# om-ai-lab/OmChat

Hardware: AMD Instinct MI355X
Metric: images/sec prefill + decode tokens/sec, OmChat-13B TP=1/8; p50 TTFT (higher is better)
Workload: dtype bf16

## Files before the change

omchat_amd/csrc/attention.hip:

```cpp
#include "kernels.h"

#include "attn_common.h"

namespace {

__device__ __forceinline__ float max3(float a, float b, float c) {
  float r;
  asm("v_max3_f32 %0, %1, %2, %3" : "=v"(r) : "v"(a), "v"(b), "v"(c));
  return r;
}
__device__ __forceinline__ float max2(float a, float b) {
  float r;
  asm("v_max_f32 %0, %1, %2" : "=v"(r) : "v"(a), "v"(b));
  return r;
}
__device__ __forceinline__ float max_xor32_raw(float v) {
  const auto r = __builtin_amdgcn_permlane32_swap(__float_as_uint(v), __float_as_uint(v), false, false);
  return max2(__uint_as_float(r[0]), __uint_as_float(r[1]));
}
__device__ __forceinline__ float max_xor16_raw(float v) {
  const auto r = __builtin_amdgcn_permlane16_swap(__float_as_uint(v), __float_as_uint(v), false, false);
  return max2(__uint_as_float(r[0]), __uint_as_float(r[1]));
}

// ... 507 lines not shown
#pragma unroll
        for (int r = 0; r < 16; ++r) mg[d * 16 + r] = o[d][r];
      mg[DB * 16] = m_run; mg[DB * 16 + 1] = l_run;
    }
    __syncthreads();
    if (kg == 1) return;
    const float m1 = mg[DB * 16], l1 = mg[DB * 16 + 1];
    const float m = max2(m_run, m1);
    const float a0 = __builtin_amdgcn_exp2f((m_run - m) * p.c), a1 = __builtin_amdgcn_exp2f((m1 - m) * p.c);
    l_run = l_run * a0 + l1 * a1;
#pragma unroll
    for (int d = 0; d < DB; ++d)
#pragma unroll
      for (int r = 0; r < 16; ++r) o[d][r] = o[d][r] * a0 + mg[d * 16 + r] * a1;
  }
  const float l = sum_xor32(l_run);
  if (wave_active && qrow < p.Sq) {
    const float inv = l > 0.f ? 1.f / l : 0.f;
    T* op = (T*)p.O + b * p.o_sb + hq * p.o_sh + (int64_t)qrow * p.o_sr + 4 * hh;
#pragma unroll
    for (int db = 0; db < DB; ++db)
#pragma unroll
      for (int g = 0; g < 4; ++g) {
        typename V8<T>::half_type h4;
#pragma unroll
        for (int r = 0; r < 4; ++r) h4[r] = fromf<T>(o[db][4 * g + r] * inv);
        *reinterpret_cast<typename V8<T>::half_type*>(op + db * 32 + g * 8) = h4;
      }
  }
}

template <typename T, bool KV8 = false, bool MASKED = false>
__global__ __launch_bounds__(64, 2) void attn_decode_kernel(AttnP p) {
  __shared__ __attribute__((aligned(256))) char Vs[KV_TILE * 256];
  const int lane = threadIdx.x, fc = lane & 15, fg = lane >> 4;
  const int split = blockIdx.x, kvh = blockIdx.y, b = blockIdx.z;
  const int n_rep = p.q_heads / p.kv_heads, hq0 = kvh * n_rep;
  const int kv_len = p.kv_len ? p.kv_len[b] : p.Skv;
#if OMCHAT_EXPERIMENTS
  if (p.dbg && split < 8 && kvh == 0 && lane == 0) atomicMax(p.dbg + 10, ~wall_clock64());
#endif
  float* wsb = p.ws + ((size_t)(b * p.q_heads + hq0 + (fc < n_rep ? fc : 0)) * p.nsplit + split) * WS_STRIDE;
  if (split * KV_TILE >= kv_len) {
    if (fc < n_rep && fg == 0) { wsb[128] = NEG_BIG; wsb[129] = 0.f; }
    return;
  }
  f32x4 o[8];
  float mx, l;
  attn_decode_tile<T, KV8, false, MASKED>(p, split, kvh, b, kv_len, Vs, lane, o, mx, l);
  if (fc < n_rep) {
#pragma unroll
    for (int dn = 0; dn < 8; ++dn) *reinterpret_cast<f32x4*>(wsb + dn * 16 + fg * 4) = o[dn];
    if (fg == 0) { wsb[128] = mx; wsb[129] = l; }
  }
#if OMCHAT_EXPERIMENTS
  if (p.dbg && kvh == 0 && lane == 0) atomicMax(p.dbg + 11, wall_clock64());
#endif
}

template <typename T, bool KLDS = false>
__global__ __launch_bounds__(64, 2) void attn_decode_multi_kernel(AttnP p) {
  typedef typename V8<T>::type frag_t;
  __shared__ __attribute__((aligned(256))) char Vs[KV_TILE * 256];
  const int lane = threadIdx.x, fc = lane & 15, fg = lane >> 4;
  const int split = blockIdx.x, kvh = blockIdx.y, b = blockIdx.z;
  const int n_rep = p.q_heads / p.kv_heads, hq0 = kvh * n_rep;
  const int kv_len = p.kv_len ? p.kv_len[b] : p.Skv;
  const int key_base = split * KV_TILE * p.tpw;
  float* wsb = p.ws + ((size_t)(b * p.q_heads + hq0 + (fc < n_rep ? fc : 0)) * p.nsplit + split) * WS_STRIDE;
  if (key_base >= kv_len) {
    if (fc < n_rep && fg == 0) { wsb[128] = NEG_BIG; wsb[129] = 0.f; }
    return;
  }
  const bool fuse = p.rope != nullptr;
  const int pp = kv_len - 1;
  const int pt = pp < p.rope_max ? pp : p.rope_max - 1;
  const T* Kg = (const T*)p.K + b * p.k_sb + kvh * p.k_sh;
  const T* Vg = (const T*)p.V + b * p.v_sb + kvh * p.v_sh;
  const T* kn = fuse ? (const T*)p.k_new + b * p.new_sb + kvh * 128 : nullptr;
  const T* vn = fuse ? (const T*)p.v_new + b * p.new_sb + kvh * 128 : nullptr;

  frag_t qf[4];
  {
    const int hh = fc < n_rep ? fc : n_rep - 1;
    const T* qp = (const T*)p.Q + b * p.q_sb + (hq0 + hh) * p.q_sh;
#pragma unroll
    for (int ds = 0; ds < 4; ++ds) qf[ds] = ld8<T>(qp + ds * 32 + fg * 8);
    if (fuse) {
#pragma unroll
      for (int ds = 0; ds < 2; ++ds) {
        const float* cs = p.rope + ((size_t)pt * 64 + ds * 32 + fg * 8) * 2;
        const frag_t lo = qf[ds], hi = qf[ds + 2];
        qf[ds] = rope_chunk<T>(lo, hi, cs, false);
        qf[ds + 2] = rope_chunk<T>(hi, lo, cs, true);
      }
    }
  }
  f32x4 o[8];
#pragma unroll
  for (int dn = 0; dn < 8; ++dn) o[dn] = (f32x4){0.f, 0.f, 0.f, 0.f};
  float m_run = NEG_BIG, l_run = 0.f;
  const int tq = fc >> 2, tp = fc & 3;
  const int vrow_lo = 4 * fg + tq;
  const int vswz = ((vrow_lo & 7) << 1);

  for (int tt = 0; tt < p.tpw; ++tt) {
// ... 790 lines not shown
  __syncthreads();
  if (g == 0) {
    float ltot = red[NWV], tot = part[0][dl];
#pragma unroll
    for (int i = 1; i < NWV; ++i) ltot += red[NWV + i];
#pragma unroll
    for (int i = 1; i < NGRP; ++i) tot += part[i][dl];
    O[pack_nb ? packed_x_index(b, h * 128 + d, pack_nb) : (size_t)(b * o_sb + h * o_sh + d)] = fromf<T>(tot / ltot);
  }
}

template <typename T>
__global__ __launch_bounds__(256) void kv_quant_kernel(const T* kc, const T* vc, unsigned char* k8, unsigned char* v8, float* ks, float* vs, int kv_heads,
                                                       int64_t c_sb, int64_t c_sh, int64_t s_sb, int64_t s_sh, const int* pos_lo, int pos0, const int* len,
                                                       int max_rows) {
  const int lane = threadIdx.x & 63, wave = threadIdx.x >> 6;
  const int r = blockIdx.x * 4 + wave;
  const int h = blockIdx.y, b = blockIdx.z;
  const int lo = pos_lo ? pos_lo[b] : pos0;
  const int pos = lo + r;
  if (r >= max_rows || (len && pos >= len[b])) return;
  const int64_t off = b * c_sb + h * c_sh + (int64_t)pos * 128 + lane * 2;
  const int64_t soff = b * s_sb + h * s_sh + pos;
#pragma unroll
  for (int which = 0; which < 2; ++which) {
    const T* src = (which ? vc : kc) + off;
    const float x0 = tof(src[0]), x1 = tof(src[1]);
    float m = fmaxf(fabsf(x0), fabsf(x1));
    m = wave_max(m);
    const float sc = m > 0.f ? m / 448.0f : 1.0f;
    const int pk = __builtin_amdgcn_cvt_pk_fp8_f32(x0 / sc, x1 / sc, 0, false);
    *reinterpret_cast<unsigned short*>((which ? v8 : k8) + off) = (unsigned short)(pk & 0xFFFF);
    if (lane == 0) (which ? vs : ks)[soff] = sc;
  }
}

}

int launch_kv_quant(int dtype, const void* kc, const void* vc, void* k8, void* v8, float* ks, float* vs, int b, int kv_heads, int64_t c_sb, int64_t c_sh,
                    int64_t s_sb, int64_t s_sh, const int* pos_lo, int pos0, const int* len, int max_rows, hipStream_t s) {
  if (b <= 0 || max_rows <= 0) return 0;
  dim3 grid(cdiv(max_rows, 4), kv_heads, b);
  if (dtype == OMCHAT_F16) hipLaunchKernelGGL(kv_quant_kernel<f16>, grid, dim3(256), 0, s, (const f16*)kc, (const f16*)vc, (unsigned char*)k8, (unsigned char*)v8,
                                              ks, vs, kv_heads, c_sb, c_sh, s_sb, s_sh, pos_lo, pos0, len, max_rows);
  else if (dtype == OMCHAT_BF16) hipLaunchKernelGGL(kv_quant_kernel<bf16>, grid, dim3(256), 0, s, (const bf16*)kc, (const bf16*)vc, (unsigned char*)k8,
                                                    (unsigned char*)v8, ks, vs, kv_heads, c_sb, c_sh, s_sb, s_sh, pos_lo, pos0, len, max_rows);
  else { omchat_set_error("launch_kv_quant: bad dtype"); return 1; }
  OM_LAUNCH_CHECK();
  return 0;
}

int g_attn_kv8_tpw = 0;
void attn_set_kv8_tpw(int v) { g_attn_kv8_tpw = v < 0 || v > 15 ? 0 : v; }
int g_attn_tpw = 0;
void attn_set_tpw(int v) { g_attn_tpw = v < 0 ? 0 : v; }
int g_merge_dg = 1;
void attn_set_merge_dg(int v) { g_merge_dg = v; }
int g_merge_mid_min = 64;
void attn_set_merge_mid_min(int v) { g_merge_mid_min = v < 1 ? 1 : v; }
int g_attn_dma = 1;
void attn_set_dma(int v) { g_attn_dma = v; }
int g_attn_dma_slots = 0;
int g_attn_dma_stages = 2;
void attn_set_dma_slots(int v) { g_attn_dma_slots = v & 255; const int st = (v >> 8) & 255; g_attn_dma_stages = st < 2 ? 2 : (st > 4 ? 4 : st); }
int g_attn_kg = 0;
void attn_set_kg(int v) { g_attn_kg = v; }
template <typename K>
static int launch_attn2(K kern, dim3 grid, int threads, int lds, hipStream_t s, const AttnP& p, PerDeviceOnce* attr_done) {
  if (attr_done->first()) OM_HIP(hipFuncSetAttribute((const void*)kern, hipFuncAttributeMaxDynamicSharedMemorySize, lds));
  hipLaunchKernelGGL(kern, grid, dim3(threads), lds, s, p);
  return 0;
}
#define OM_LAUNCH_ATTN2(KERN, GRID, THREADS, LDS)                                     \
  do { static PerDeviceOnce done_; const int rc_ = launch_attn2((KERN), (GRID), (THREADS), (LDS), s, p, &done_); if (rc_) return rc_; } while (0)
int g_attn_peel = 1;
void attn_set_peel(int v) { g_attn_peel = v; }
int g_attn_mha_xcd = 1;
void attn_set_mha_xcd(int v) { g_attn_mha_xcd = v; }
int g_attn_hsplit = -1;
void attn_set_hsplit(int v) { g_attn_hsplit = v; }
int g_attn_dma_rot = 0;
void attn_set_dma_rot(int v) { g_attn_dma_rot = v; }
int g_attn_klds = 0;
void attn_set_klds(int v) { g_attn_klds = v; }
int g_attn_v2 = 1;
void attn_set_v2(int v) { g_attn_v2 = v; }

namespace {
template <typename T>
__global__ __launch_bounds__(128) void attn_uniform_rows_kernel(AttnP p) {
  const int h = blockIdx.x, b = blockIdx.y, d = threadIdx.x;
  const int start = p.kv_start[b];
  if (start <= 0) return;
  const int kvh = h / (p.q_heads / p.kv_heads);
  const T* V = (const T*)p.V + b * p.v_sb + kvh * p.v_sh + d;
  const float w = rnd<T>(1.0f / (float)p.Skv);
  float acc = 0.f;
  for (int j = 0; j < p.Skv; ++j) acc += w * tof(V[(int64_t)j * p.v_sr]);
  const T o = fromf<T>(acc);
  T* O = (T*)p.O + b * p.o_sb + h * p.o_sh + d;
  for (int i = 0; i < start && i < p.Sq; ++i) O[(int64_t)i * p.o_sr] = o;
}
}

int launch_attn_uniform_rows(int dtype, const AttnArgs& a, hipStream_t s) {
  OM_CHECK(a.kv_start && (a.head_dim == 0 || a.head_dim == 128), "uniform rows: left-padded batch (kv_start), head dim 128");
// ... 101 lines not shown
  return (size_t)batch * q_heads * cdiv(max_len, KV_TILE) * WS_STRIDE * sizeof(float);
}

static void kv8_plan(int batch, int kv_heads, int L, bool masked, int* tpw, int* nw) {
  *tpw = 1; *nw = 1;
  if (masked) return;
  const long waves1 = (long)cdiv(L, KV_TILE) * kv_heads * batch;
  if (g_attn_kv8_tpw > 0) { *tpw = g_attn_kv8_tpw & 7; *nw = (g_attn_kv8_tpw & 8) ? 4 : 1; }
  else {
    *tpw = waves1 >= 2L * device_cus() ? 3 : 1;
    const int n4 = cdiv(L, 12 * KV_TILE);
    if (*tpw == 3 && n4 <= 64 && (long)n4 * kv_heads * batch >= device_cus() / 2) *nw = 4;
  }
  if (*tpw < 1 || *tpw > 4) *tpw = 1;
  if (*tpw != 3) *nw = 1;
}
int g_attn_kv8_fuse = 1;
void attn_set_kv8_fuse(int v) { g_attn_kv8_fuse = v; }
bool attn_decode_kv8_fuses_rope(int batch, int kv_heads, int L, bool masked) {
  int tpw, nw;
  kv8_plan(batch, kv_heads, L, masked, &tpw, &nw);
  const long waves = (long)cdiv(L, KV_TILE * tpw * nw) * nw * kv_heads * batch;
  return g_attn_kv8_fuse && tpw == 3 && waves <= 4L * device_cus();
}

struct MergeDone { unsigned* flags = nullptr; unsigned epoch = 0; int mode = 0; unsigned long long* dbg = nullptr; };
template <typename T>
static void launch_merge(const float* ws, int nsplit, int q_heads, int rows, const int* kv_len, int L, float c, void* O, int64_t o_sb, int64_t o_sh,
                         int pack_nb, int split_keys, hipStream_t s, const MergeDone& done = MergeDone{}) {
  const dim3 mgrid(q_heads, rows);
  if (nsplit > g_merge_mid_min && nsplit <= 256) {
    if (g_merge_dg == 2) hipLaunchKernelGGL((attn_merge_mid_kernel<T, 4, 2>), dim3(q_heads, rows, 2), dim3(512), 0, s, ws, nsplit, q_heads, kv_len, L, c, (T*)O, o_sb, o_sh, pack_nb, split_keys);
    else hipLaunchKernelGGL((attn_merge_mid_kernel<T, 4, 1>), mgrid, dim3(512), 0, s, ws, nsplit, q_heads, kv_len, L, c, (T*)O, o_sb, o_sh, pack_nb, split_keys);
  } else if (nsplit > 256 && nsplit <= 1024) {
    if (g_merge_dg >= 1) hipLaunchKernelGGL((attn_merge_mid_kernel<T, 8, 4>), dim3(q_heads, rows, 4), dim3(1024), 0, s, ws, nsplit, q_heads, kv_len, L, c, (T*)O, o_sb, o_sh, pack_nb, split_keys);
    else hipLaunchKernelGGL((attn_merge_mid_kernel<T, 8, 1>), mgrid, dim3(1024), 0, s, ws, nsplit, q_heads, kv_len, L, c, (T*)O, o_sb, o_sh, pack_nb, split_keys);
  } else {
    hipLaunchKernelGGL(attn_merge_kernel<T>, mgrid, dim3(128), 0, s, ws, nsplit, q_heads, kv_len, L, c, (T*)O, o_sb, o_sh, pack_nb, split_keys,
                       done.flags, done.epoch, done.mode, done.dbg);
  }
}

int launch_attn_merge(int dtype, const float* ws, int nsplit, int q_heads, int rows, const int* kv_len, int L, float scale, void* O, int split_keys,
                      hipStream_t s) {
  OM_CHECK(ws && O && nsplit > 0 && q_heads > 0 && rows > 0 && L > 0 && split_keys > 0, "launch_attn_merge: null or empty argument");
  const float c = scale * 1.4426950408889634f;
  if (dtype == OMCHAT_F16) launch_merge<f16>(ws, nsplit, q_heads, rows, kv_len, L, c, O, (int64_t)q_heads * 128, 128, 0, split_keys, s);
  else if (dtype == OMCHAT_BF16) launch_merge<bf16>(ws, nsplit, q_heads, rows, kv_len, L, c, O, (int64_t)q_heads * 128, 128, 0, split_keys, s);
  else { omchat_set_error("launch_attn_merge: bad dtype"); return 1; }
  OM_LAUNCH_CHECK();
  return 0;
}

struct DecodeForm { bool masked, kv8, kv8_fuse, dma; int tpw, kv8_nw, dma_lds, nsplit, split_keys; };
template <typename T>
static void launch_decode_form(const AttnDecodeArgs& a, const DecodeForm& f, dim3 grid, const AttnP& p, hipStream_t s) {
  if (f.masked && f.kv8) hipLaunchKernelGGL((attn_decode_kernel<T, true, true>), grid, dim3(64), 0, s, p);
  else if (f.masked) hipLaunchKernelGGL((attn_decode_kernel<T, false, true>), grid, dim3(64), 0, s, p);
  else if (f.kv8 && f.tpw == 2) hipLaunchKernelGGL((attn_decode_kv8_walk_kernel<T, 2, 1>), grid, dim3(64), 0, s, p);
  else if (f.kv8_fuse && f.kv8_nw == 4) hipLaunchKernelGGL((attn_decode_kv8_walk_kernel<T, 3, 4, true>), grid, dim3(256), 0, s, p);
  else if (f.kv8_fuse) hipLaunchKernelGGL((attn_decode_kv8_walk_kernel<T, 3, 1, true>), grid, dim3(64), 0, s, p);
  else if (f.kv8 && f.tpw == 3 && f.kv8_nw == 4) hipLaunchKernelGGL((attn_decode_kv8_walk_kernel<T, 3, 4>), grid, dim3(256), 0, s, p);
  else if (f.kv8 && f.tpw == 3) hipLaunchKernelGGL((attn_decode_kv8_walk_kernel<T, 3, 1>), grid, dim3(64), 0, s, p);
  else if (f.kv8 && f.tpw == 4) hipLaunchKernelGGL((attn_decode_kv8_walk_kernel<T, 4, 1>), grid, dim3(64), 0, s, p);
  else if (f.kv8) hipLaunchKernelGGL((attn_decode_kernel<T, true>), grid, dim3(64), 0, s, p);
  else if (f.dma && g_attn_dma_stages == 2) hipLaunchKernelGGL((attn_decode_dma_kernel<T, 2>), grid, dim3(64), f.dma_lds, s, p);
  else if (f.dma && g_attn_dma_stages == 3) hipLaunchKernelGGL((attn_decode_dma_kernel<T, 3>), grid, dim3(64), f.dma_lds, s, p);
  else if (f.dma) hipLaunchKernelGGL((attn_decode_dma_kernel<T, 4>), grid, dim3(64), f.dma_lds, s, p);
  else if (f.tpw > 1 && g_attn_klds) hipLaunchKernelGGL((attn_decode_multi_kernel<T, true>), grid, dim3(64), 0, s, p);
  else if (f.tpw > 1) hipLaunchKernelGGL((attn_decode_multi_kernel<T, false>), grid, dim3(64), 0, s, p);
  else hipLaunchKernelGGL((attn_decode_kernel<T, false>), grid, dim3(64), 0, s, p);
  launch_merge<T>(a.ws, f.nsplit, a.q_heads, a.batch, a.kv_len, a.L, p.c, a.O, a.o_sb, a.o_sh, a.o_pack_nb, f.split_keys, s,
                  MergeDone{a.done_flags, a.done_epoch, a.done_mode, a.done_dbg});
}

int launch_attn_decode(int dtype, const AttnDecodeArgs& a, hipStream_t s) {
  OM_CHECK(a.q_heads % a.kv_heads == 0 && a.q_heads / a.kv_heads <= 16, "group size must be <= 16");
  OM_CHECK(a.L > 0 && a.batch > 0, "empty attention");
  const bool kv8 = a.k_scale != nullptr;
  const long waves1 = (long)cdiv(a.L, KV_TILE) * a.kv_heads * a.batch;
  int tpw = kv8 ? 1 : (waves1 >= 6144 ? 4 : (waves1 >= 3072 ? 2 : 1));
  if (g_attn_tpw > 0 && !kv8) tpw = g_attn_tpw;
  int kv8_nw = 1;
  if (kv8) kv8_plan(a.batch, a.kv_heads, a.L, a.key_mask != nullptr, &tpw, &kv8_nw);
  if (a.key_mask) tpw = 1;
  const long tiles32 = (long)cdiv(a.L, DMA_TILE) * a.kv_heads * a.batch;
  const bool dma = g_attn_dma && !kv8 && !a.key_mask && a.k_sr == 128 && a.v_sr == 128 && (g_attn_tpw > 1 || (g_attn_tpw == 0 && tiles32 >= 6L * device_cus()));
  int dma_slots = g_attn_dma_slots;
  if (!dma_slots) {
    const int pairs = a.kv_heads * a.batch, tpw4 = cdiv(cdiv(a.L, DMA_TILE), std::max(1, 4 * device_cus() / pairs));
    dma_slots = (pairs >= 16 && tpw4 >= 4 && tpw4 <= 8 && tiles32 < 32L * device_cus()) ? 4 : 2;
  }
  int split_keys = KV_TILE * tpw * kv8_nw;
  if (dma) {
    const int slots = dma_slots * device_cus(), pairs = a.kv_heads * a.batch;
    const int tiles = cdiv(a.L, DMA_TILE);
    const int ns_target = std::max(1, slots / pairs);
    tpw = std::max(2, cdiv(tiles, ns_target));
    split_keys = DMA_TILE * tpw;
  }
  const int nsplit = cdiv(a.L, split_keys);
  OM_CHECK(a.ws && a.ws_bytes >= attn_decode_ws_bytes(a.batch, a.q_heads, a.L), "workspace too small");
  AttnP p{a.Q, a.K, a.V, nullptr, a.q_sb, a.q_sh, 0, a.k_sb, a.k_sh, a.k_sr, a.v_sb, a.v_sh, a.v_sr, 0, 0, 0,
          a.kv_len, nullptr, a.q_heads, a.kv_heads, 1, a.L, 0, 0, nsplit, a.scale * 1.4426950408889634f, a.ws,
          a.rope, a.pos, a.k_new, a.v_new, a.new_sb, (void*)a.K, (void*)a.V, a.rope_max, a.k_scale, a.v_scale, a.scale_sb, a.scale_sh, tpw,
          a.key_mask, a.mask_sb};
#if OMCHAT_EXPERIMENTS
  p.dbg = a.done_dbg;
#endif
  OM_CHECK(!a.key_mask || (((kv8 && !a.rope) || (!kv8 && a.rope && a.pos)) && !a.kv_len && a.mask_sb % 64 == 0 && a.mask_sb >= a.L),
           "masked decode: fused RoPE with explicit positions (16-bit cache) or rows appended beforehand (e4m3 cache), uniform length, mask rows padded to a multiple of 64");
  const bool kv8_fuse = kv8 && a.rope != nullptr;
  OM_CHECK(!kv8 || a.v_scale, "fp8 KV cache: both scale arrays");
  OM_CHECK(!kv8_fuse || (tpw == 3 && a.k_new && a.v_new && a.k16_w && a.v16_w && !a.key_mask),
           "fp8 KV cache with fused RoPE: the walking form only (attn_decode_kv8_fuses_rope), raw k / v rows and the 16-bit caches to append to");
  OM_CHECK(!a.rope || (a.k_new && a.v_new), "fused RoPE decode needs k_new and v_new (kv_len == null: every sequence holds exactly L keys)");
  OM_CHECK(a.o_pack_nb == 0 || (a.batch <= 16 * a.o_pack_nb && a.o_sh == 128 && a.q_heads % 1 == 0), "packed output: batch <= 16 * NB, head stride 128");
  if (kv8_fuse) { p.k_cache_w = a.k16_w; p.v_cache_w = a.v16_w; }
  if (dma) p.causal = g_attn_dma_rot == 1;
  const int dma_lds = std::min(65536, std::max(g_attn_dma_stages * 16384, (160 / dma_slots) * 1024));
  dim3 grid(nsplit, a.kv_heads, a.batch);
  if (a.done_flags && (a.batch != 1 || nsplit > 64 || nsplit > g_merge_mid_min)) { omchat_set_error("launch_attn_decode: completion flags exist for the one-round-trip merge only (batch 1, <= 64 splits)"); return 1; }
  const DecodeForm f{a.key_mask != nullptr, kv8, kv8_fuse, dma, tpw, kv8_nw, dma_lds, nsplit, split_keys};
  if (dtype == OMCHAT_F16) launch_decode_form<f16>(a, f, grid, p, s);
  else if (dtype == OMCHAT_BF16) launch_decode_form<bf16>(a, f, grid, p, s);
  else { omchat_set_error("launch_attn_decode: bad dtype"); return 1; }
  OM_LAUNCH_CHECK();
  return 0;
}

template <typename T, int NW, bool EXT = false, bool SHR = false, bool SFX = false>
__global__ __launch_bounds__(NW * 64) void attn_verify_kernel(AttnP p) {
  typedef typename V8<T>::type frag_t;
  constexpr int PER = 16 / NW;
  __shared__ __attribute__((aligned(256))) char Ks[KV_TILE * 256];
  __shared__ __attribute__((aligned(256))) char Vs[KV_TILE * 256];
  const int lane = threadIdx.x & 63, w = threadIdx.x >> 6, fc = lane & 15, fg = lane >> 4;
  const int kvh = blockIdx.y;
  const int n_rep = p.q_heads / p.kv_heads, hq0 = kvh * n_rep;
  int split = blockIdx.x;
  int t0 = EXT ? (int)blockIdx.z * 16 : 0;
  int NT = EXT ? min(16, p.Sq - t0) : p.Sq, L = p.q_pos0 + t0, Lt = EXT ? L + NT : p.Skv;
  int key_base = split * KV_TILE * p.tpw, ntile = p.tpw;
  int64_t row_off_k = 0, row_off_v = 0, row_off_new = 0;
  if constexpr (SHR) {
    const int nss = p.nsplit - p.shr_nsp, x = (int)blockIdx.x - p.shr_nsp;
    const bool pre = x < 0;
    const int j = pre ? 0 : x / nss, ss = pre ? 0 : x - j * nss;
    t0 = (int)blockIdx.z * p.Sq + j;
    NT = pre ? p.Sq : 1;
    const int len = p.kv_len ? p.kv_len[t0] : p.shr_L;
    if (!pre) { split = p.shr_nsp + ss; key_base = p.Skv + ss * KV_TILE; ntile = 1; }
    Lt = pre ? p.Skv : len;
    L = pre ? 0x3fffffff : len - 1;
    row_off_k = t0 * p.k_sb; row_off_v = t0 * p.v_sb; row_off_new = t0 * p.new_sb;
  }
  if constexpr (SFX) {
    const int x = (int)blockIdx.x - p.shr_nsp;
    if (x < 0) {
      t0 = (int)blockIdx.z * 16;
      if (t0 >= p.shr_L) return;
      NT = min(16, p.shr_L - t0);
      Lt = p.Skv; L = 0x3fffffff;
    } else {
      const int cps = (p.Sq + 15) >> 4, j = (int)blockIdx.z / cps, c16 = ((int)blockIdx.z - j * cps) * 16;
      t0 = j * p.Sq + c16;
      NT = min(16, p.Sq - c16);
      L = p.Skv + c16;
      Lt = min(L + NT, p.kv_len[j]);
      split = p.shr_nsp + x; key_base = p.Skv + x * KV_TILE * p.q_pos0; ntile = p.q_pos0;
      row_off_k = j * p.k_sb; row_off_v = j * p.v_sb;
    }
  }
  const int R = NT * n_rep;
  const bool active = 16 * w < R;
  const int r = min(16 * w + fc, R - 1), t = r / n_rep, hh = r - t * n_rep;
// ... 300 lines not shown
```

omchat_amd/csrc/capi.hip:

```cpp
#include "kernels.h"
#include <stdlib.h>
#include "../../include/omchat_hip.h"
#include <math.h>
#include <vector>

#define S(x) ((hipStream_t)(x))
#if OMCHAT_EXPERIMENTS
int g_launch_any_order = 0;
#endif

extern "C" int omchat_op_gemm(int dtype, const void* A, int lda, const void* W, int ldw, void* C, int ldc, int M, int N, int K,
                              const void* bias, const void* ls, const void* resid, int ldr, int epi, int force_tile, void* stream) {
  GemmArgs g{A, lda, W, ldw, C, ldc, M, N, K, bias, ls, resid, ldr, epi, force_tile, nullptr, 0, -1};
  return launch_gemm(dtype, g, S(stream));
}

extern "C" int omchat_op_gemm_fused(int dtype, const void* A, int lda, const void* W, int ldw, void* C, int ldc, int M, int N, int K,
                                    const void* bias, const void* ls, const void* resid, int ldr, int epi, int force_tile, const float* row_scale,
                                    const float* rs_stats, int rs_ld, int rs_nslots, int rs_dim, float rs_eps,
                                    float* stats, int stats_ld, int* nslots, void* stream) {
  GemmArgs g{A, lda, W, ldw, C, ldc, M, N, K, bias, ls, resid, ldr, epi, force_tile, nullptr, 0, -1};
  g.row_scale = row_scale; g.stats = stats; g.stats_ld = stats_ld; g.stats_nslots = nslots;
  g.rs_stats = rs_stats; g.rs_ld = rs_ld; g.rs_nslots = rs_nslots; g.rs_dim = rs_dim; g.rs_eps = rs_eps;
  return launch_gemm(dtype, g, S(stream));
// ... 21 lines not shown
  a.V = (const char*)qkv + (size_t)2 * H * 128 * 2; a.v_sb = a.q_sb; a.v_sh = 128; a.v_sr = row;
  a.O = out; a.o_sb = (int64_t)Sq * H * 128; a.o_sh = 128; a.o_sr = (int64_t)H * 128;
  a.batch = B; a.q_heads = H; a.kv_heads = H; a.Sq = Sq; a.Skv = Sq; a.kv_len = nullptr; a.causal = 0; a.q_pos0 = 0;
  a.scale = 1.0f;
  a.qn_sumsq = sumsq; a.qn_stride = stride; a.qn_dim = dim; a.qn_w = wq; a.qn_eps = eps; a.qn_scale = q_scale;
  return launch_attn_prefill(dtype, a, S(stream));
}

extern "C" int omchat_op_set_tuning(int key, int value) {
  const char* allow = getenv("OMCHAT_ALLOW_TUNING");
  if (!allow || allow[0] != '1') {
    omchat_set_error("omchat_op_set_tuning: process-global test / measurement hook; set OMCHAT_ALLOW_TUNING=1 to use it (see include/omchat_hip.h)");
    return 1;
  }
  if (key == 0) { gemm_set_skew(value); return 0; }
  if (key == 1) { gemv_set_force_mfma(value); return 0; }
  if (key == 5) { gemm_set_autotune(value); return 0; }
  if (key == 4) { model_set_ar_min_rows(value); return 0; }
  if (key == 6) { model_set_pack_replica(value); return 0; }
  if (key == 8) { attn_set_v2(value); return 0; }
  if (key == 9) { model_set_fuse_peer_norm(value); return 0; }
  if (key == 10) { attn_set_tpw(value); return 0; }
  if (key == 11) { gemv_set_no_xs(value); return 0; }
  if (key == 12) { attn_set_klds(value); return 0; }
  if (key == 25) { attn_set_dma(value); return 0; }
  if (key == 26) { attn_set_dma_slots(value); return 0; }
  if (key == 27) { attn_set_dma_rot(value); return 0; }
  if (key == 28) { gemv_set_skew(value); return 0; }
  if (key == 29) { model_set_tp_f32(value); return 0; }
  if (key == 30) { attn_set_hsplit(value); return 0; }
  if (key == 33) { attn_set_mha_xcd(value); return 0; }
  if (key == 16) { gemv_set_norm_loop(value); return 0; }
  if (key == 17) { gemv_set_rows_balance(value); return 0; }
  if (key == 19) { attn_set_merge_mid_min(value); return 0; }
  if (key == 21) { attn_set_merge_dg(value); return 0; }
  if (key == 13) { gemm_set_persist(value); return 0; }
  if (key == 14) { model_set_norm_in_gemv(value); return 0; }
  if (key == 22) { model_set_fuse_attn_oproj(value); return 0; }
  if (key == 23) { model_set_decode_layer(value); return 0; }
  if (key == 24) { gemv_set_dyn(value); return 0; }
  if (key == 34) { gemv_set_shard_shapes(value); return 0; }
  if (key == 35) { model_set_shard_as_tp1(value); return 0; }
  if (key == 36) { attn_set_kg(value); return 0; }
  if (key == 37) { gemm_set_wide_store(value); return 0; }
  if (key == 43) { gemm_set_skip_dead(value); return 0; }
  if (key == 44) { model_set_vit_fused(value); return 0; }
  if (key == 45) { model_set_tp_sp(value); return 0; }
  if (key == 46) { attn_set_peel(value); return 0; }
  if (key == 47) { attn_set_kv8_tpw(value); return 0; }
  if (key == 48) { attn_set_kv8_fuse(value); return 0; }
  if (key == 49) { model_set_extend_attn(value); return 0; }
  if (key == 50) { model_set_x12_roles(value); return 0; }
  if (key == 51) { model_set_suffix_attn(value); return 0; }
  if (key == 38) { gemv_set_gu_rr(value); return 0; }
  if (key == 39) { gemv_set_longk_direct(value); return 0; }
  if (key == 40) { norm_set_wave(value); return 0; }
#if OMCHAT_EXPERIMENTS
  if (key == 41) { g_launch_any_order = value; return 0; }
  if (key == 42) { model_set_ao_oproj(value); return 0; }
#endif
  omchat_set_error("omchat_op_set_tuning: unknown key");
  return 1;
}

extern "C" int omchat_allreduce_noop(void*, void*, size_t, int, void*) { return 0; }

extern "C" int omchat_gemm_tune_load(const char* path) { OM_CHECK(path, "null path"); return gemm_tune_load(path); }
extern "C" int omchat_gemm_tune_dump(const char* path) { OM_CHECK(path, "null path"); return gemm_tune_dump(path); }
extern "C" long omchat_gemm_tune_runs(void) { return gemm_tune_runs(); }

extern "C" size_t omchat_op_gemm_sk_ws(void) { return gemm_sk_ws_bytes(); }

extern "C" int omchat_op_gemm_sk(int dtype, const void* A, int lda, const void* W, int ldw, void* C, int ldc, int M, int N, int K,
                                 const void* bias, const void* ls, const void* resid, int ldr, int epi, int force_tile, void* ws,
                                 size_t ws_bytes, int stream_k, void* stream) {
  GemmArgs g{A, lda, W, ldw, C, ldc, M, N, K, bias, ls, resid, ldr, epi, force_tile, ws, ws_bytes, stream_k};
  return launch_gemm(dtype, g, S(stream));
}

extern "C" int omchat_op_gemv(int dtype, const void* X, int ldx, const void* W, int ldw, void* Y, int ldy, int b, int N, int K,
                              const void* bias, const void* resid, int ldr, int epi, int out_f32, void* stream) {
  GemvArgs g{X, ldx, W, ldw, Y, ldy, b, N, K, bias, resid, ldr, epi, out_f32};
  return launch_gemv(dtype, g, S(stream));
}

extern "C" int omchat_op_gemv_norm(int dtype, const void* X, const void* W, int ldw, void* Y, int N, int K, const void* norm_w, float eps,
                                   const void* bias, int epi, int out_f32, void* stream) {
  OM_CHECK(X && W && Y && norm_w, "null argument");
  GemvArgs g{X, K, W, ldw, Y, N, 1, N, K, bias, nullptr, 0, epi, out_f32};
  g.norm_w = norm_w; g.norm_eps = eps;
  return launch_gemv(dtype, g, S(stream));
}

extern "C" int omchat_op_gemv_packed(int dtype, const void* X, int ldx, const void* W, int ldw, void* Y, int ldy, int b, int N, int K,
                                     const void* bias, int epi, int out_f32, int ksplit, int w_packed, int y_packed, void* stream) {
  OM_CHECK(b >= 1 && b <= 32 && K % 64 == 0, "1 <= b <= 32, K % 64 == 0");
  const int NB = b > 16 ? 2 : 1;
  void *xp = nullptr, *wp = nullptr;
  OM_HIP(hipMalloc(&xp, (size_t)NB * 16 * K * 2));
  int rc = launch_pack_x(dtype, X, ldx, b, K, xp, S(stream));
  if (rc == 0 && w_packed) {
    if (hipMalloc(&wp, (size_t)N * K * 2) != hipSuccess) { hipFree(xp); omchat_set_error("hipMalloc failed"); return 2; }
    rc = launch_pack_w(dtype, W, ldw, N, K, wp, S(stream));
  }
  if (rc == 0) {
    GemvArgs g{xp, K, w_packed ? wp : W, ldw, Y, ldy, b, N, K, bias, nullptr, 0, epi, out_f32, ksplit, 0, nullptr, 1, w_packed, y_packed};
// ... 963 lines not shown
```

omchat_amd/csrc/kernels.h:

```cpp
#pragma once
#ifndef OMCHAT_EXPERIMENTS
#define OMCHAT_EXPERIMENTS 0
#endif
#include "common.h"
#if OMCHAT_EXPERIMENTS
#include <hip/hip_ext.h>
extern int g_launch_any_order;
#undef hipLaunchKernelGGL
#define hipLaunchKernelGGL(kernelName, numBlocks, numThreads, memPerBlock, streamId, ...)                                                      \
  do {                                                                                                                                         \
    if (g_launch_any_order)                                                                                                                    \
      hipExtLaunchKernelGGL((kernelName), dim3(numBlocks), dim3(numThreads), (memPerBlock), (streamId), nullptr, nullptr, hipExtAnyOrderLaunch, \
                            __VA_ARGS__);                                                                                                      \
    else                                                                                                                                       \
      hipLaunchKernelGGLInternal((kernelName), numBlocks, numThreads, memPerBlock, streamId, __VA_ARGS__);                                     \
  } while (0)
#endif

enum {
  EPI_NONE = 0,
  EPI_GELU = 1,
  EPI_LS_RESID = 2,
  EPI_RESID = 3,
  EPI_SWIGLU = 4,
// ... 91 lines not shown
int gemm_tune_dump(const char* path);
long gemm_tune_runs();
void model_set_ar_min_rows(int v);
void model_set_tp_f32(int v);
void model_set_pack_replica(int v);
void model_set_norm_in_gemv(int v);
void model_set_vit_fused(int v);
void model_set_tp_sp(int v);
int launch_fold_cols(int dtype, const void* W, const void* n, void* out, int rows, int cols, hipStream_t s);

int launch_layernorm(int dtype, const void* x, int ldx, const void* w, const void* b, void* y, int ldy, int rows, int H, float eps, hipStream_t stream);
int launch_rmsnorm(int dtype, const void* x, int ldx, const void* w, void* y, int ldy, int rows, int H, float eps, hipStream_t s, int pack_nb = 0);
int launch_rmsnorm_q8(int dtype, const void* x, int ldx, const void* w, void* y8, int ldy, float* scale, int rows, int H, float eps, hipStream_t s);
int launch_quant_rows_q8(int dtype, const void* x, int ldx, void* y8, int ldy, float* scale, int rows, int H, hipStream_t s);
int launch_resid_rmsnorm(int dtype, void* x, int ldx, const float* part, int ks, const void* w, void* xn, int ldn, int rows, int H, float eps,
                         hipStream_t s, int pack_nb = 0);
int launch_resid16_norm(int dtype, void* x, int ldx, const void* y, int ldy, const void* w, const void* b, void* xn, int ldn, int rows, int H, float eps,
                        hipStream_t s);
int launch_vit_qknorm(int dtype, void* qkv, int ld, const void* wq, const void* wk, int rows, int C, int C_total,
                      float eps, float q_scale, const float* sumsq_in, hipStream_t s, int only_k = 0);
int launch_vit_qk_sumsq(int dtype, const void* qkv, int ld, int rows, int C, float* sumsq_out, hipStream_t s);
int launch_vit_knorm_slots(int dtype, void* k, int ld, const void* wk, int rows, int C, int C_total, float eps, const float* stats, int stats_ld, int nslots,
                           float* sumsq_q, hipStream_t s);
struct AttnArgs {
  const void* Q; int64_t q_sb, q_sh, q_sr;
  const void* K; int64_t k_sb, k_sh, k_sr;
  const void* V; int64_t v_sb, v_sh, v_sr;
  void* O; int64_t o_sb, o_sh, o_sr;
  int batch, q_heads, kv_heads;
  int Sq, Skv;
  const int* kv_len;
  const int* kv_start;
  int causal;
  int q_pos0;
  float scale;
  int head_dim;
  const float* qn_sumsq = nullptr; int qn_stride = 0, qn_dim = 0; const void* qn_w = nullptr; float qn_eps = 0.f, qn_scale = 1.f;
};
int launch_attn_prefill(int dtype, const AttnArgs& a, hipStream_t s);
int launch_attn_uniform_rows(int dtype, const AttnArgs& a, hipStream_t s);
void attn_set_v2(int v);
void model_set_fuse_peer_norm(int v);
void attn_set_tpw(int v);
void attn_set_klds(int v);
void attn_set_dma(int v);
void attn_set_dma_slots(int v);
void attn_set_dma_rot(int v);
void attn_set_hsplit(int v);
void attn_set_mha_xcd(int v);
void attn_set_kg(int v);
void attn_set_peel(int v);
void attn_set_kv8_tpw(int v);
void attn_set_kv8_fuse(int v);
void model_set_extend_attn(int v);
void model_set_x12_roles(int v);
void model_set_suffix_attn(int v);
int gemv_x12_default_forms();
bool attn_decode_kv8_fuses_rope(int batch, int kv_heads, int L, bool masked);
void attn_set_merge_mid_min(int v);
void attn_set_merge_dg(int v);
void gemv_set_norm_loop(int v);
void gemv_set_dyn(int v);
void gemv_set_skew(int v);
void gemv_set_rows_balance(int v);
void gemv_set_no_xs(int v);
void gemv_set_shard_shapes(int v);
void gemv_set_gu_rr(int v);
void gemv_set_longk_direct(int v);
void norm_set_wave(int v);
void model_set_ao_oproj(int v);
int gemv_get_shard_shapes();

struct AttnOperands {
  const void* Q; int64_t q_sb, q_sh;
  const void* K; int64_t k_sb, k_sh, k_sr;
  const void* V; int64_t v_sb, v_sh, v_sr;
  void* O; int64_t o_sb, o_sh;
  int q_heads, kv_heads;
  float scale;
  float* ws; size_t ws_bytes;
  const float* rope; int rope_max;
  const void* k_new; const void* v_new; int64_t new_sb;
  int o_pack_nb;
};

struct AttnDecodeArgs : AttnOperands {
  int batch;
  int L;
  const int* kv_len;
  const int* pos;
  const float* k_scale; const float* v_scale; int64_t scale_sb, scale_sh;
  void* k16_w = nullptr; void* v16_w = nullptr;
  const unsigned char* key_mask; int64_t mask_sb;
  unsigned* done_flags = nullptr; unsigned done_epoch = 0; int done_mode = 0;
  unsigned long long* done_dbg = nullptr;
};
int launch_kv_quant(int dtype, const void* kc, const void* vc, void* k8, void* v8, float* ks, float* vs, int b, int kv_heads, int64_t c_sb, int64_t c_sh,
                    int64_t s_sb, int64_t s_sh, const int* pos_lo, int pos0, const int* len, int max_rows, hipStream_t s);
size_t attn_decode_ws_bytes(int batch, int q_heads, int max_len);
int launch_attn_decode(int dtype, const AttnDecodeArgs& a, hipStream_t s);
int launch_attn_merge(int dtype, const float* ws, int nsplit, int q_heads, int rows, const int* kv_len, int L, float scale, void* O, int split_keys,
                      hipStream_t s);

enum AttnBlockMode { ATTN_VERIFY = 0, ATTN_EXTEND, ATTN_SHARED, ATTN_SUFFIX };
struct AttnBlockArgs : AttnOperands {
  int mode;
// ... 211 lines not shown
```

Before: 391.8.

## Add 4-wave split-K decode attention kernel for batch-1 bf16 KV path

Adds a 256-thread decode attention kernel that spreads one KV tile across four wavefronts. Each wave loads a quarter of the K rows and V chunks, stages K, V and roped Q in LDS, and computes its own slice of the output head dimension. RoPE on the new key and the cache write-back are fused in. It is enabled by default for batch 1 on the non-kv8, non-masked, non-DMA, tpw=1 path, and is meant to cut per-block latency of the single-wave decode kernel. In exchange it uses more LDS and a block barrier.

```diff
diff --git a/omchat_amd/csrc/attention.hip b/omchat_amd/csrc/attention.hip
--- a/omchat_amd/csrc/attention.hip
+++ b/omchat_amd/csrc/attention.hip
@@ -583,6 +583,163 @@
 #pragma unroll
     for (int dn = 0; dn < 8; ++dn) *reinterpret_cast<f32x4*>(wsb + dn * 16 + fg * 4) = o[dn];
     if (fg == 0) { wsb[128] = mx; wsb[129] = l; }
+  }
+#if OMCHAT_EXPERIMENTS
+  if (p.dbg && kvh == 0 && lane == 0) atomicMax(p.dbg + 11, wall_clock64());
+#endif
+}
+
+template <typename T>
+__global__ __launch_bounds__(256) void attn_decode_4w_kernel(AttnP p) {
+  typedef typename V8<T>::type frag_t;
+  __shared__ __attribute__((aligned(256))) char Ks[KV_TILE * 256];
+  __shared__ __attribute__((aligned(256))) char Vs[KV_TILE * 256];
+  __shared__ __attribute__((aligned(16))) char Qs[4 * 64 * 16];
+  const int w = __builtin_amdgcn_readfirstlane(threadIdx.x >> 6);
+  const int lane = threadIdx.x & 63, fc = lane & 15, fg = lane >> 4;
+  const int split = blockIdx.x, kvh = blockIdx.y, b = blockIdx.z;
+  const int n_rep = p.q_heads / p.kv_heads, hq0 = kvh * n_rep;
+  const int kv_len = p.kv_len ? p.kv_len[b] : p.Skv;
+#if OMCHAT_EXPERIMENTS
+  if (p.dbg && split < 8 && kvh == 0 && threadIdx.x == 0) atomicMax(p.dbg + 10, ~wall_clock64());
+#endif
+  float* wsb = p.ws + ((size_t)(b * p.q_heads + hq0 + (fc < n_rep ? fc : 0)) * p.nsplit + split) * WS_STRIDE;
+  const int key0 = split * KV_TILE;
+  if (key0 >= kv_len) {
+    if (w == 0 && fc < n_rep && fg == 0) { wsb[128] = NEG_BIG; wsb[129] = 0.f; }
+    return;
+  }
+  const bool fuse = p.rope != nullptr;
+  const int pp = kv_len - 1;
+  const int pt = pp < p.rope_max ? (pp > 0 ? pp : 0) : p.rope_max - 1;
+  const T* Kg = (const T*)p.K + b * p.k_sb + kvh * p.k_sh;
+  const T* Vg = (const T*)p.V + b * p.v_sb + kvh * p.v_sh;
+  const T* kn = fuse ? (const T*)p.k_new + b * p.new_sb + kvh * 128 : nullptr;
+  const T* vn = fuse ? (const T*)p.v_new + b * p.new_sb + kvh * 128 : nullptr;
+
+  const int hh = fc < n_rep ? fc : n_rep - 1;
+  const T* qp = (const T*)p.Q + b * p.q_sb + (hq0 + hh) * p.q_sh;
+  const frag_t q_own = ld8<T>(qp + w * 32 + fg * 8), q_par = ld8<T>(qp + (w ^ 2) * 32 + fg * 8);
+  float csq[16];
+  {
+    const f32x4* cs = reinterpret_cast<const f32x4*>(fuse ? p.rope + ((size_t)pt * 64 + (w & 1) * 32 + fg * 8) * 2 : (const float*)p.Q);
+#pragma unroll
+    for (int q4 = 0; q4 < 4; ++q4) { const f32x4 v = cs[q4]; csq[4 * q4] = v[0]; csq[4 * q4 + 1] = v[1]; csq[4 * q4 + 2] = v[2]; csq[4 * q4 + 3] = v[3]; }
+  }
+  const frag_t kn_own = ld8<T>((fuse ? kn : (const T*)p.Q) + fc * 8), kn_par = ld8<T>((fuse ? kn : (const T*)p.Q) + (fc ^ 8) * 8);
+  float csk[16];
+  {
+    const f32x4* cs = reinterpret_cast<const f32x4*>(fuse ? p.rope + ((size_t)pt * 64 + (fc & 7) * 8) * 2 : (const float*)p.Q);
+#pragma unroll
+    for (int q4 = 0; q4 < 4; ++q4) { const f32x4 v = cs[q4]; csk[4 * q4] = v[0]; csk[4 * q4 + 1] = v[1]; csk[4 * q4 + 2] = v[2]; csk[4 * q4 + 3] = v[3]; }
+  }
+  __builtin_amdgcn_sched_barrier(0);
+
+  frag_t kr[4];
+#pragma unroll
+  for (int i = 0; i < 4; ++i) {
+    const int key = key0 + 16 * w + 4 * i + fg;
+    const int kc = fuse ? (key < pp ? key : (pp > 0 ? pp - 1 : 0)) : (key < kv_len ? key : kv_len - 1);
+    kr[i] = ld8s<T>(Kg + (int64_t)kc * p.k_sr + fc * 8);
+  }
+  const int vrr = lane >> 2, vrl = (vrr & 8) | ((vrr & 3) << 1) | ((vrr >> 2) & 1), vch = 4 * w + (lane & 3);
+  frag_t vr[4];
+#pragma unroll
+  for (int i = 0; i < 4; ++i) {
+    const int key = key0 + 16 * i + vrl;
+    const bool fresh = fuse && key >= pp;
+    const T* src = fresh ? vn : Vg + (int64_t)(key < kv_len ? key : kv_len - 1) * p.v_sr;
+    vr[i] = ld8s<T>(src + vch * 8);
+  }
+  __builtin_amdgcn_sched_barrier(0);
+
+  *reinterpret_cast<frag_t*>(Qs + (w * 64 + lane) * 16) = fuse ? rope_chunk<T>(q_own, q_par, csq, w >= 2) : q_own;
+  if (fuse && key0 + 16 * w + 15 >= pp) {
+    const frag_t rot = rope_chunk<T>(kn_own, kn_par, csk, fc >= 8);
+#pragma unroll
+    for (int i = 0; i < 4; ++i) {
+      const int key = key0 + 16 * w + 4 * i + fg;
+      kr[i] = key >= pp ? rot : kr[i];
+      if (key == pp) st8<T>((T*)p.k_cache_w + b * p.k_sb + kvh * p.k_sh + (int64_t)pp * p.k_sr + fc * 8, kr[i]);
+    }
+  }
+#pragma unroll
+  for (int i = 0; i < 4; ++i) {
+    const int row = 16 * w + 4 * i + fg;
+    *reinterpret_cast<frag_t*>(Ks + row * 256 + ((fc ^ (row & 15)) << 4)) = kr[i];
+  }
+  __syncthreads();
+  frag_t qf[4];
+#pragma unroll
+  for (int ds = 0; ds < 4; ++ds) qf[ds] = *reinterpret_cast<const frag_t*>(Qs + (ds * 64 + lane) * 16);
+
+  f32x4 s[4];
+#pragma unroll
+  for (int kt = 0; kt < 4; ++kt) {
+    frag_t kf[4];
+#pragma unroll
+    for (int ds = 0; ds < 4; ++ds) kf[ds] = *reinterpret_cast<const frag_t*>(Ks + (kt * 16 + fc) * 256 + (((ds * 4 + fg) ^ fc) << 4));
+    s[kt] = (f32x4){0.f, 0.f, 0.f, 0.f};
+#pragma unroll
+    for (int ds = 0; ds < 4; ++ds) s[kt] = mfma16(kf[ds], qf[ds], s[kt]);
+  }
+  float mx = NEG_BIG;
+#pragma unroll
+  for (int kt = 0; kt < 4; ++kt)
+#pragma unroll
+    for (int r = 0; r < 4; ++r) {
+      const float v = key0 + kt * 16 + 4 * fg + r < kv_len ? s[kt][r] : NEG_BIG;
+      s[kt][r] = v;
+      mx = fmaxf(mx, v);
+    }
+  mx = max_xor32(max_xor16(mx));
+  const float mc = mx * p.c;
+  float psum = 0.f;
+  frag_t pf[2];
+#pragma unroll
+  for (int ks = 0; ks < 2; ++ks) {
+    typedef float f32x8 __attribute__((ext_vector_type(8)));
+    f32x8 e;
+#pragma unroll
+    for (int j = 0; j < 8; ++j) {
+      e[j] = __builtin_amdgcn_exp2f(fmaf(s[2 * ks + (j >> 2)][j & 3], p.c, -mc));
+      psum += e[j];
+    }
+    pf[ks] = __builtin_convertvector(e, frag_t);
+  }
+  const float l = sum_xor32(sum_xor16(psum));
+
+#pragma unroll
+  for (int i = 0; i < 4; ++i) {
+    const int row = 16 * i + vrl;
+    *reinterpret_cast<frag_t*>(Vs + row * 256 + ((vch ^ ((row & 7) << 1)) << 4)) = vr[i];
+    if (fuse && key0 + row == pp)
+      st8<T>((T*)p.v_cache_w + b * p.v_sb + kvh * p.v_sh + (int64_t)pp * p.v_sr + vch * 8, vr[i]);
+  }
+  __builtin_amdgcn_wave_barrier(); asm volatile("s_waitcnt lgkmcnt(0)" ::: "memory"); __builtin_amdgcn_wave_barrier();
+
+  const int tq = fc >> 2, tp = fc & 3;
+  const int vrow_lo = 4 * fg + tq;
+  const int vswz = ((vrow_lo & 7) << 1);
+  f32x4 o[2];
+#pragma unroll
+  for (int dd = 0; dd < 2; ++dd) o[dd] = (f32x4){0.f, 0.f, 0.f, 0.f};
+#pragma unroll
+  for (int ks = 0; ks < 2; ++ks)
+#pragma unroll
+    for (int dd = 0; dd < 2; ++dd) {
+      const int ch = (2 * (2 * w + dd) + (tp >> 1)) ^ vswz;
+      const char* a0 = Vs + (ks * 32 + vrow_lo) * 256 + (ch << 4) + 8 * (tp & 1);
+      const s16x4 lo = tr_read(a0);
+      const s16x4 hi = tr_read(a0 + 16 * 256);
+      typedef short s16x8 __attribute__((ext_vector_type(8)));
+      const s16x8 cat = __builtin_shufflevector(lo, hi, 0, 1, 2, 3, 4, 5, 6, 7);
+      o[dd] = mfma16(__builtin_bit_cast(frag_t, cat), pf[ks], o[dd]);
+    }
+  if (fc < n_rep) {
+#pragma unroll
+    for (int dd = 0; dd < 2; ++dd) *reinterpret_cast<f32x4*>(wsb + (2 * w + dd) * 16 + fg * 4) = o[dd];
+    if (w == 0 && fg == 0) { wsb[128] = mx; wsb[129] = l; }
   }
 #if OMCHAT_EXPERIMENTS
   if (p.dbg && kvh == 0 && lane == 0) atomicMax(p.dbg + 11, wall_clock64());
@@ -1479,6 +1636,8 @@
 
 int g_attn_kv8_tpw = 0;
 void attn_set_kv8_tpw(int v) { g_attn_kv8_tpw = v < 0 || v > 15 ? 0 : v; }
+int g_attn_4w = 1;
+void attn_set_4w(int v) { g_attn_4w = v < 0 || v > 2 ? 1 : v; }
 int g_attn_tpw = 0;
 void attn_set_tpw(int v) { g_attn_tpw = v < 0 ? 0 : v; }
 int g_merge_dg = 1;
@@ -1686,7 +1845,7 @@
   return 0;
 }
 
-struct DecodeForm { bool masked, kv8, kv8_fuse, dma; int tpw, kv8_nw, dma_lds, nsplit, split_keys; };
+struct DecodeForm { bool masked, kv8, kv8_fuse, dma, w4; int tpw, kv8_nw, dma_lds, nsplit, split_keys; };
 template <typename T>
 static void launch_decode_form(const AttnDecodeArgs& a, const DecodeForm& f, dim3 grid, const AttnP& p, hipStream_t s) {
   if (f.masked && f.kv8) hipLaunchKernelGGL((attn_decode_kernel<T, true, true>), grid, dim3(64), 0, s, p);
@@ -1703,6 +1862,7 @@
   else if (f.dma) hipLaunchKernelGGL((attn_decode_dma_kernel<T, 4>), grid, dim3(64), f.dma_lds, s, p);
   else if (f.tpw > 1 && g_attn_klds) hipLaunchKernelGGL((attn_decode_multi_kernel<T, true>), grid, dim3(64), 0, s, p);
   else if (f.tpw > 1) hipLaunchKernelGGL((attn_decode_multi_kernel<T, false>), grid, dim3(64), 0, s, p);
+  else if (f.w4) hipLaunchKernelGGL(attn_decode_4w_kernel<T>, grid, dim3(256), 0, s, p);
   else hipLaunchKernelGGL((attn_decode_kernel<T, false>), grid, dim3(64), 0, s, p);
   launch_merge<T>(a.ws, f.nsplit, a.q_heads, a.batch, a.kv_len, a.L, p.c, a.O, a.o_sb, a.o_sh, a.o_pack_nb, f.split_keys, s,
                   MergeDone{a.done_flags, a.done_epoch, a.done_mode, a.done_dbg});
@@ -1755,7 +1915,8 @@
   const int dma_lds = std::min(65536, std::max(g_attn_dma_stages * 16384, (160 / dma_slots) * 1024));
   dim3 grid(nsplit, a.kv_heads, a.batch);
   if (a.done_flags && (a.batch != 1 || nsplit > 64 || nsplit > g_merge_mid_min)) { omchat_set_error("launch_attn_decode: completion flags exist for the one-round-trip merge only (batch 1, <= 64 splits)"); return 1; }
-  const DecodeForm f{a.key_mask != nullptr, kv8, kv8_fuse, dma, tpw, kv8_nw, dma_lds, nsplit, split_keys};
+  const bool w4 = !kv8 && !a.key_mask && !dma && tpw == 1 && (g_attn_4w == 2 || (g_attn_4w == 1 && a.batch == 1));
+  const DecodeForm f{a.key_mask != nullptr, kv8, kv8_fuse, dma, w4, tpw, kv8_nw, dma_lds, nsplit, split_keys};
   if (dtype == OMCHAT_F16) launch_decode_form<f16>(a, f, grid, p, s);
   else if (dtype == OMCHAT_BF16) launch_decode_form<bf16>(a, f, grid, p, s);
   else { omchat_set_error("launch_attn_decode: bad dtype"); return 1; }
diff --git a/omchat_amd/csrc/capi.hip b/omchat_amd/csrc/capi.hip
--- a/omchat_amd/csrc/capi.hip
+++ b/omchat_amd/csrc/capi.hip
@@ -97,6 +97,7 @@
   if (key == 49) { model_set_extend_attn(value); return 0; }
   if (key == 50) { model_set_x12_roles(value); return 0; }
   if (key == 51) { model_set_suffix_attn(value); return 0; }
+  if (key == 52) { attn_set_4w(value); return 0; }
   if (key == 38) { gemv_set_gu_rr(value); return 0; }
   if (key == 39) { gemv_set_longk_direct(value); return 0; }
   if (key == 40) { norm_set_wave(value); return 0; }
diff --git a/omchat_amd/csrc/kernels.h b/omchat_amd/csrc/kernels.h
--- a/omchat_amd/csrc/kernels.h
+++ b/omchat_amd/csrc/kernels.h
@@ -167,6 +167,7 @@
 void attn_set_peel(int v);
 void attn_set_kv8_tpw(int v);
 void attn_set_kv8_fuse(int v);
+void attn_set_4w(int v);
 void model_set_extend_attn(int v);
 void model_set_x12_roles(int v);
 void model_set_suffix_attn(int v);
```

Result: faster. 396.4, median of 6 (+1.2%).
